# SingleRust/single-algebra

Hardware: AMD Instinct MI355X
Metric: sparse_pca_fit_transform_algorithmic_throughput (higher is better)
Workload: dtype f32

## Files before the change

### single-algebra_amd/csrc/common.h

```cpp
#pragma once
#include <hip/hip_runtime.h>

#include <atomic>
#include <cstdint>
#include <cstdio>
#include <stdexcept>
#include <string>
#include <vector>

#include "../../include/sapca.h"
#include "switches.h"

namespace sapca {

struct Error : std::runtime_error {
  sapca_status code;
  Error(sapca_status c, const std::string& m) : std::runtime_error(m), code(c) {}
};

#define SAPCA_HIP(expr)                                                                        \
  do {                                                                                         \
    hipError_t e_ = (expr);                                                                    \
    if (e_ != hipSuccess)                                                                      \
      throw ::sapca::Error(SAPCA_ERR_HIP, std::string(#expr) + ": " + hipGetErrorString(e_)); \
  } while (0)

#define SAPCA_CHECK(cond, code, msg)                 \
  do {                                               \
    if (!(cond)) throw ::sapca::Error((code), (msg)); \
  } while (0)

inline int64_t round_up(int64_t x, int64_t q) { return (x + q - 1) / q * q; }

struct DevBuf {
  void* p = nullptr;
  size_t cap = 0;
  DevBuf() = default;
  DevBuf(const DevBuf&) = delete;
  DevBuf& operator=(const DevBuf&) = delete;
  ~DevBuf() { release(); }
  void release() {
    if (p) (void)hipFree(p);
    p = nullptr;
    cap = 0;
  }
  void* ensure(size_t bytes) {
    if (bytes > cap) {
      release();
      size_t want = bytes + bytes / 16 + 256;
      hipError_t e = hipMalloc(&p, want);
      if (e != hipSuccess) {
        p = nullptr;
        throw Error(SAPCA_ERR_NOMEM, std::string("hipMalloc(") + std::to_string(want) + "): " + hipGetErrorString(e));
      }
      cap = want;
    }
    return p;
  }
  template <typename U>
  U* as(size_t count) { return static_cast<U*>(ensure(count * sizeof(U))); }
// ... 48 lines not shown
      cap = bytes;
    }
    return p;
  }
};

struct TiledOp {
  bool valid = false;
  int64_t rows = 0, cols = 0, total_entries = 0;
  int ldp = 0;
  int elem = 4;
  int tc = 0, nct = 0;
  int nrb = 0;
  int block_rows = 0;
  int nsplit = 1, tiles_per_split = 0;
  int tile_bytes = 0;
  int64_t max_chunk = 0;
  const int32_t* blk_row0 = nullptr;
  int64_t mid_row0 = -1;
  const uint32_t* row_perm = nullptr;
  const int64_t* chunk_off = nullptr;
  const uint32_t* wave_off = nullptr;
  const uint8_t* steps = nullptr;
  const void* ent = nullptr;
  bool dq = false;
  const uint32_t* dq_info = nullptr;
};
struct TiledBuffers {
  DevBuf blk, steps, wave_off, chunk_off, ent, tmp, misc, perm, lens, dq_info, bounds;
  DevBuf seg;
  DevBuf quad_off;
  DevBuf raw;
  PinnedBuf host;
  hipStream_t aux = nullptr;
  hipEvent_t aux_fork = nullptr, aux_join = nullptr;
  TiledBuffers() = default;
  TiledBuffers(const TiledBuffers&) = delete;
  TiledBuffers& operator=(const TiledBuffers&) = delete;
  ~TiledBuffers() {
    if (aux) { (void)hipStreamSynchronize(aux); (void)hipStreamDestroy(aux); }
    if (aux_fork) (void)hipEventDestroy(aux_fork);
    if (aux_join) (void)hipEventDestroy(aux_join);
  }
};

struct Stream {
  hipStream_t s = nullptr;
  bool owned = false;
};

struct EventTimer {
  bool enabled = false;
  hipStream_t s = nullptr;
  std::vector<std::pair<hipEvent_t, hipEvent_t>> pool;
  size_t used = 0;
  struct Span { size_t i; };
  void begin_collect(hipStream_t st, bool on) {
    enabled = on;
    s = st;
    used = 0;
  }
  int start() {
    if (!enabled) return -1;
    if (used == pool.size()) {
      hipEvent_t a, b;
      SAPCA_HIP(hipEventCreate(&a));
      SAPCA_HIP(hipEventCreate(&b));
      pool.emplace_back(a, b);
    }
    SAPCA_HIP(hipEventRecord(pool[used].first, s));
    return (int)used++;
  }
  void stop(int i) {
    if (i >= 0) SAPCA_HIP(hipEventRecord(pool[i].second, s));
  }
  double ms(int i) {
    if (i < 0) return 0.0;
    float t = 0;
    SAPCA_HIP(hipEventElapsedTime(&t, pool[i].first, pool[i].second));
    return t;
  }
  ~EventTimer() {
    for (auto& p : pool) {
      (void)hipEventDestroy(p.first);
      (void)hipEventDestroy(p.second);
    }
  }
};

}
```

### single-algebra_amd/csrc/dense.hip

```cpp
#include "kernels.h"

#include <algorithm>
#include <cmath>
#include <vector>

namespace sapca {
namespace k {

namespace {

constexpr int WAVE = 64;
typedef double d4 __attribute__((ext_vector_type(4)));

__device__ inline d4 mfma_f64(double a, double b, d4 c) { return __builtin_amdgcn_mfma_f64_16x16x4f64(a, b, c, 0, 0, 0); }

template <typename T, int NT>
__global__ void __launch_bounds__(256)
gram_kernel(const T* __restrict__ P, int64_t rows, int ld, double* __restrict__ slabs, const T* __restrict__ Pb = nullptr) {
  constexpr int NPAIR = NT * (NT + 1) / 2;
  extern __shared__ double lds[];
  const int lane = threadIdx.x & (WAVE - 1);
  const int wave = threadIdx.x / WAVE;
  const int g = lane >> 4, c = lane & 15;
  d4 acc[NPAIR];
// ... 121 lines not shown
    const double2 a = *reinterpret_cast<const double2*>(p);
    const double2 b = *reinterpret_cast<const double2*>(p + 2);
    out[0] = a.x; out[1] = a.y; out[2] = b.x; out[3] = b.y;
  }
  __device__ static inline void store(double* p, const double v[4]) {
    *reinterpret_cast<double2*>(p) = make_double2(v[0], v[1]);
    *reinterpret_cast<double2*>(p + 2) = make_double2(v[2], v[3]);
  }
};

template <typename T, int NT, bool SRC, int W>
__device__ __forceinline__ void gramv_wave(T* P, int64_t rows, int ld, double* __restrict__ slab, double* lds,
                                           const PanelSource<T>& src, const T* __restrict__ wgt, int want_sum, int lane, int wave) {
  constexpr int NPAIR = NT * (NT + 1) / 2;
  constexpr bool SPLIT = NT > 6;
  constexpr int MINE = SPLIT ? (NPAIR - W + 3) / 4 : NPAIR;
  constexpr int NH = NT / 4;
  const int g = lane >> 4, c = lane & 15;
  const bool owner = !SPLIT || W == 0;
  d4 acc[MINE];
#pragma unroll
  for (int p = 0; p < MINE; ++p) acc[p] = d4{0, 0, 0, 0};
  double cs[NT];
#pragma unroll
  for (int t = 0; t < NT; ++t) cs[t] = 0;
  const int64_t stride = SPLIT ? (int64_t)gridDim.x * 4 : (int64_t)gridDim.x * 16;
  int64_t r0 = SPLIT ? (int64_t)blockIdx.x * 4 : ((int64_t)blockIdx.x * 4 + wave) * 4;
  auto mma = [&](const T (&x)[NT], double wr) {
    double v[NT];
#pragma unroll
    for (int t = 0; t < NT; ++t) v[t] = (double)x[t];
    if (want_sum && owner) {
#pragma unroll
      for (int t = 0; t < NT; ++t) cs[t] += wr * v[t];
    }
    int p = 0, mine = 0;
#pragma unroll
    for (int ta = 0; ta < NT; ++ta)
#pragma unroll
      for (int tb = ta; tb < NT; ++tb) {
        if (!SPLIT || p % 4 == W) {
          acc[mine] = mfma_f64(v[ta], v[tb], acc[mine]);
          ++mine;
        }
        ++p;
      }
  };
  if constexpr (SRC) {
    T sv[NT];
    if (src.mu) {
#pragma unroll
      for (int hh = 0; hh < NH; ++hh) Four<T>::load(src.sv + 64 * hh + 4 * c, &sv[4 * hh]);
    }
    for (; r0 < rows; r0 += stride) {
      const int64_t r = r0 + g;
      T x[NT];
#pragma unroll
      for (int t = 0; t < NT; ++t) x[t] = (T)0;
      double wr = 0;
      if (r < rows) {
        const T* p = src.parts + r * ld + 4 * c;
#pragma unroll
        for (int hh = 0; hh < NH; ++hh) Four<T>::load(p + 64 * hh, &x[4 * hh]);
        for (int sp = 1; sp < src.nsplit; ++sp) {
          T y[NT];
#pragma unroll
          for (int hh = 0; hh < NH; ++hh) Four<T>::load(p + sp * src.slab_stride + 64 * hh, &y[4 * hh]);
#pragma unroll
          for (int t = 0; t < NT; ++t) x[t] += y[t];
        }
        if (src.mu) {
          const T m = src.mu[r];
#pragma unroll
          for (int t = 0; t < NT; ++t) x[t] -= m * sv[t];
        }
        if (owner) {
#pragma unroll
          for (int hh = 0; hh < NH; ++hh) Four<T>::store(P + r * ld + 64 * hh + 4 * c, &x[4 * hh]);
        }
        wr = wgt ? (double)wgt[r] : 1.0;
      }
      mma(x, wr);
    }
  } else {
    constexpr int D = NT == 4 ? 4 : 2;
    T buf[D][NT];
    double wb[D];
    auto fetch = [&](int64_t r, T (&out)[NT], double& wr) {
      if (r < rows) {
#pragma unroll
        for (int hh = 0; hh < NH; ++hh) Four<T>::load(P + r * ld + 64 * hh + 4 * c, &out[4 * hh]);
        wr = (want_sum && wgt) ? (double)wgt[r] : 1.0;
      } else {
#pragma unroll
        for (int t = 0; t < NT; ++t) out[t] = (T)0;
        wr = 0;
      }
    };
#pragma unroll
    for (int d = 0; d < D; ++d) fetch(r0 + d * stride + g, buf[d], wb[d]);
    for (; r0 < rows; r0 += D * stride) {
#pragma unroll
      for (int d = 0; d < D; ++d) {
        T x[NT];
#pragma unroll
        for (int t = 0; t < NT; ++t) x[t] = buf[d][t];
        const double wr = wb[d];
        fetch(r0 + (d + D) * stride + g, buf[d], wb[d]);
        mma(x, wr);
      }
    }
  }
  if (want_sum && owner) {
#pragma unroll
    for (int t = 0; t < NT; ++t) {
      cs[t] += __shfl_xor(cs[t], 16);
      cs[t] += __shfl_xor(cs[t], 32);
    }
  }
  if constexpr (SPLIT) {
#pragma unroll
    for (int q = 0; q < MINE; ++q)
#pragma unroll
      for (int reg = 0; reg < 4; ++reg) slab[((W + 4 * q) * 4 + reg) * WAVE + lane] = acc[q][reg];
    if (owner && g == 0) {
#pragma unroll
      for (int t = 0; t < NT; ++t) slab[NPAIR * 256 + 16 * t + c] = want_sum ? cs[t] : 0.0;
    }
  } else {
    double* lsum = lds + NPAIR * 256;
    for (int w = 0; w < 4; ++w) {
      if (wave == w) {
#pragma unroll
        for (int p = 0; p < NPAIR; ++p)
#pragma unroll
          for (int reg = 0; reg < 4; ++reg) {
            double* dst = lds + (p * 4 + reg) * WAVE + lane;
            if (w == 0) *dst = acc[p][reg]; else *dst += acc[p][reg];
          }
        if (g == 0) {
#pragma unroll
          for (int t = 0; t < NT; ++t) {
            double* dst = lsum + 16 * t + c;
            if (w == 0) *dst = cs[t]; else *dst += cs[t];
          }
        }
      }
      __syncthreads();
    }
    for (int i = threadIdx.x; i < NPAIR * 256 + 16 * NT; i += blockDim.x) slab[i] = lds[i];
  }
}

template <typename T, int NT, bool SRC>
__global__ void __launch_bounds__(256)
gramv_kernel(T* P, int64_t rows, int ld, double* __restrict__ slabs, PanelSource<T> src, const T* __restrict__ wgt, int want_sum) {
  constexpr int NPAIR = NT * (NT + 1) / 2;
  extern __shared__ double lds[];
  const int lane = threadIdx.x & (WAVE - 1), wave = threadIdx.x / WAVE;
  double* slab = slabs + (int64_t)blockIdx.x * (NPAIR * 256 + 16 * NT);
  if constexpr (NT > 6) {
    switch (wave) {
      case 0: gramv_wave<T, NT, SRC, 0>(P, rows, ld, slab, lds, src, wgt, want_sum, lane, wave); break;
      case 1: gramv_wave<T, NT, SRC, 1>(P, rows, ld, slab, lds, src, wgt, want_sum, lane, wave); break;
      case 2: gramv_wave<T, NT, SRC, 2>(P, rows, ld, slab, lds, src, wgt, want_sum, lane, wave); break;
      default: gramv_wave<T, NT, SRC, 3>(P, rows, ld, slab, lds, src, wgt, want_sum, lane, wave); break;
    }
  } else {
    gramv_wave<T, NT, SRC, 0>(P, rows, ld, slab, lds, src, wgt, want_sum, lane, wave);
  }
}

template <typename T>
__global__ void materialize_kernel(T* P, int64_t rows, int ld, PanelSource<T> src) {
  const int64_t total = rows * ld;
  int64_t i = (int64_t)blockIdx.x * blockDim.x + threadIdx.x;
  const int64_t stride = (int64_t)gridDim.x * blockDim.x;
  for (; i < total; i += stride) {
    T x = src.parts[i];
    for (int sp = 1; sp < src.nsplit; ++sp) x += src.parts[(int64_t)sp * src.slab_stride + i];
    if (src.mu) x -= src.mu[i / ld] * src.sv[i % ld];
    P[i] = x;
  }
}

template <typename T>
__global__ void rinv_tvec_kernel(const double* __restrict__ Rinv, int l, int ld, const double* __restrict__ wsum, T* __restrict__ vec) {
  const int j = blockIdx.x * blockDim.x + threadIdx.x;
  if (j >= ld) return;
  double s = 0;
  if (j < l)
    for (int i = 0; i <= j; ++i) s += Rinv[(size_t)i * ld + j] * wsum[i];
  vec[j] = (T)s;
}

__global__ void __launch_bounds__(256)
gram_reduce_kernel(const double* __restrict__ slabs, int nslabs, int nt, int ld, double* __restrict__ G, int vtiles = 0,
                   double* __restrict__ wsum = nullptr) {
  __shared__ double part[16][17];
  const int npair = nt * (nt + 1) / 2;
  const int slab_len = npair * 256 + (vtiles ? 16 * nt : 0);
  const int e = threadIdx.x & 15, grp = threadIdx.x >> 4;
  const int i = blockIdx.x * 16 + e;
  double sum = 0;
  if (i < slab_len)
    for (int b = grp; b < nslabs; b += 16) sum += slabs[(int64_t)b * slab_len + i];
  part[grp][e] = sum;
  __syncthreads();
  if (grp != 0 || i >= slab_len) return;
  sum = 0;
#pragma unroll
  for (int g2 = 0; g2 < 16; ++g2) sum += part[g2][e];
  if (i >= npair * 256) {
    const int t = (i - npair * 256) / 16, c = (i - npair * 256) % 16;
    if (wsum) wsum[vcol(t, c)] = sum;
    return;
  }
  int p = i / 256, rem = i % 256, reg = rem / 64, lane = rem % 64;
  int ta = 0;
  while (p >= nt - ta) { p -= nt - ta; ++ta; }
  const int tb = ta + p;
  const int row = vtiles ? vcol(ta, (lane >> 4) + 4 * reg) : 16 * ta + (lane >> 4) + 4 * reg;
  const int col = vtiles ? vcol(tb, lane & 15) : 16 * tb + (lane & 15);
  G[row * ld + col] = sum;
  G[col * ld + row] = sum;
}

__global__ void __launch_bounds__(256)
chol_inv_kernel(const double* __restrict__ G, int l, int ld, double* __restrict__ R, double* __restrict__ Rinv,
                int* __restrict__ info) {
  extern __shared__ double a[];
  const int st = l + 1;
  double* dinv = a + (size_t)l * st;
  __shared__ int bad;
  __shared__ double floor_s;
  const int tid = threadIdx.x;
  const int ti = tid >> 4, tj = tid & 15;
  if (tid == 0) bad = 0;
  for (int i = tid; i < l * l; i += blockDim.x) a[(i / l) * st + (i % l)] = G[(i / l) * ld + (i % l)];
  __syncthreads();
  if (tid == 0) {
    double scale = 0;
    for (int i = 0; i < l; ++i) scale = fmax(scale, fabs(a[i * st + i]));
    floor_s = scale * 1e-13 + 1e-300;
  }
  __syncthreads();
  for (int kk = 0; kk < l; ++kk) {
    if (tid == 0) {
      double v = a[kk * st + kk];
      if (!(v > floor_s)) { v = floor_s; bad += 1; }
      v = sqrt(v);
      a[kk * st + kk] = v;
      dinv[kk] = 1.0 / v;
    }
    __syncthreads();
    const double inv = dinv[kk];
    for (int j = kk + 1 + tid; j < l; j += blockDim.x) a[kk * st + j] *= inv;
    __syncthreads();
    for (int i = kk + 1 + ti; i < l; i += 16) {
// ... 317 lines not shown
  }
  __syncthreads();
  chol_inv_core<false>(B0, B2, dinvs, nb2, floor_s, bad);
#pragma unroll
  for (int u = 0; u < 16; ++u) {
    const int e = t + u * 256, r = e >> 6, c = e & 63;
    const bool in = r < l2 && c < l2 && c >= r;
    R[(size_t)(CHN + r) * LD + CHN + c] = in ? B0[c * CHP + r] : 0.0;
    Rinv[(size_t)(CHN + r) * LD + CHN + c] = in ? B2[c * CHP + r] : 0.0;
  }
  __syncthreads();
  for (int blk = wave; blk < 16; blk += 4) {
    const int I = blk >> 2, J = blk & 3;
    const d4 acc = mm_block(B3 + I * CHB * CHP + J * CHB, CHP, 1, B1 + J * CHB * CHP + J * CHB, CHP, 1, 4 - J, lane);
#pragma unroll
    for (int reg = 0; reg < 4; ++reg) B0[(I * CHB + g4 + 4 * reg) * CHP + J * CHB + i16] = acc[reg];
  }
  __syncthreads();
  for (int blk = wave; blk < 16; blk += 4) {
    const int I = blk >> 2, J = blk & 3;
    const d4 acc = mm_block(B2 + I * CHB * CHP, CHP, 1, B0 + J * CHB, CHP, 1, I + 1, lane);
#pragma unroll
    for (int reg = 0; reg < 4; ++reg) B3[(I * CHB + g4 + 4 * reg) * CHP + J * CHB + i16] = -acc[reg];
  }
  __syncthreads();
#pragma unroll
  for (int u = 0; u < 16; ++u) {
    const int e = t + u * 256, r = e >> 6, c = e & 63;
    Rinv[(size_t)r * LD + CHN + c] = c < l2 ? B3[c * CHP + r] : 0.0;
  }
  if (t == 0 && bad) atomicAdd(info, bad);
}

template <typename T> struct Quad;
template <> struct Quad<float> {
  __device__ static inline void load(const float* p, double out[4]) {
    const float4 v = *reinterpret_cast<const float4*>(p);
    out[0] = v.x; out[1] = v.y; out[2] = v.z; out[3] = v.w;
  }
};
template <> struct Quad<double> {
  __device__ static inline void load(const double* p, double out[4]) {
    const double2 a = *reinterpret_cast<const double2*>(p);
    const double2 b = *reinterpret_cast<const double2*>(p + 2);
    out[0] = a.x; out[1] = a.y; out[2] = b.x; out[3] = b.y;
  }
};

template <typename T, int NTO, int THREADS = 256>
__global__ void __launch_bounds__(THREADS, THREADS == 512 ? 4 : 1)
panel_gemm_kernel(const T* P, int64_t rows, int ld, const double* __restrict__ M, int ldo, T* out, int ldp_stride, int ldm_stride,
                  int ldo_stride, int accumulate, int upper, int ncols_out) {
  extern __shared__ double Ms[];
  for (int i = threadIdx.x; i < ld * ldo; i += blockDim.x) Ms[i] = M[(i / ldo) * ldm_stride + (i % ldo)];
  __syncthreads();
  const int lane = threadIdx.x & (WAVE - 1);
  const int wave = threadIdx.x / WAVE;
  const int i = lane & 15, g = lane >> 4;
  const int nt = ld / 16;
  const int64_t ntiles = (rows + 15) / 16;
  constexpr int WPB = THREADS / WAVE;
  for (int64_t tile = (int64_t)blockIdx.x * WPB + wave; tile < ntiles; tile += (int64_t)gridDim.x * WPB) {
    const int64_t r0 = tile * 16;
    const bool row_ok = r0 + i < rows;
    const T* prow = P + (row_ok ? (r0 + i) : 0) * ldp_stride + 4 * g;
    d4 acc[NTO];
#pragma unroll
    for (int tb = 0; tb < NTO; ++tb) acc[tb] = d4{0, 0, 0, 0};
    for (int j = 0; j < nt; ++j) {
      double a4[4] = {0, 0, 0, 0};
      if (row_ok) Quad<T>::load(prow + 16 * j, a4);
#pragma unroll
      for (int e = 0; e < 4; ++e) {
        const double* brow = Ms + (16 * j + 4 * g + e) * ldo + i;
#pragma unroll
        for (int tb = 0; tb < NTO; ++tb)
          if (!upper || tb + upper - 1 >= j) acc[tb] = mfma_f64(a4[e], brow[16 * tb], acc[tb]);
      }
    }
#pragma unroll
    for (int tb = 0; tb < NTO; ++tb)
#pragma unroll
      for (int reg = 0; reg < 4; ++reg) {
        const int64_t r = r0 + g + 4 * reg;
        if (r < rows && 16 * tb + i < ncols_out) {
          T* o = out + r * ldo_stride + 16 * tb + i;
          *o = accumulate ? (T)((double)*o + acc[tb][reg]) : (T)acc[tb][reg];
        }
      }
  }
}

constexpr int EIG_THREADS = 1024;
constexpr int EIG_MAX_L = 112;
constexpr int EIG_MAX_SWEEPS = 40;

__device__ __forceinline__ int eig_tri(int i, int j, int l) {
  return i * l - (i * (i - 1)) / 2 + (j - i);
}

__global__ void __launch_bounds__(EIG_THREADS)
sym_eig_jacobi_kernel(const double* __restrict__ G, int l, int ld, int k, int ldk, double* __restrict__ M, double* __restrict__ sigma_out,
                      int* __restrict__ status) {
  extern __shared__ double eig_lds[];
  const int L = (l + 1) & ~1;
  const int np = L / 2;
  const int vs = l | 1;
// ... 325 lines not shown

inline int grid_for(int64_t work_items, int block, int cap = 4096) {
  int64_t g = (work_items + block - 1) / block;
  if (g < 1) g = 1;
  if (g > cap) g = cap;
  return (int)g;
}

template <typename T>
static void colsum_f64(const T* P, int64_t rows, int ld, const T* w, double* out, double* partial, hipStream_t s) {
  int by = 256 / ld;
  if (by < 1) by = 1;
  int nblocks = (int)((rows + by * 8 - 1) / (by * 8));
  if (nblocks > 1024) nblocks = 1024;
  if (nblocks < 1) nblocks = 1;
  hipLaunchKernelGGL((colsum_partial_kernel<T>), dim3(nblocks), dim3(ld, by), (size_t)by * ld * sizeof(double), s, P, rows, ld, w, partial);
  hipLaunchKernelGGL((colsum_final_kernel<double>), dim3(ld), dim3(64), 0, s, partial, nblocks, ld, out);
}

template <typename T, int NT>
void launch_gram(const T* P, int64_t rows, int ld, double* slabs, int nblocks, hipStream_t s) {
  constexpr int NPAIR = NT * (NT + 1) / 2;
  if constexpr (NT >= 7) {
    hipLaunchKernelGGL((gram_split_kernel<T, NT>), dim3(nblocks), dim3(256), 0, s, P, rows, ld, slabs, (const T*)nullptr);
    return;
  }
  const size_t lds = (size_t)NPAIR * 256 * sizeof(double);
  static LdsAttrState attr;
  if (lds > 48 * 1024) ensure_dynamic_lds(reinterpret_cast<const void*>(&gram_kernel<T, NT>), lds, attr);
  hipLaunchKernelGGL((gram_kernel<T, NT>), dim3(nblocks), dim3(256), lds, s, P, rows, ld, slabs);
}

template <typename T, int NTO>
void launch_panel_gemm(const T* P, int64_t rows, int ld, const double* M, int ldo, T* out, hipStream_t s, int ldp_stride = 0,
                       int ldm_stride = 0, int ldo_stride = 0, int accumulate = 0, int upper = 0, int ncols_out = 0) {
  if (ncols_out <= 0 || ncols_out > ldo) ncols_out = ldo;
  const size_t lds = (size_t)ld * ldo * sizeof(double);
  static LdsAttrState attr;
  if (lds > 48 * 1024) ensure_dynamic_lds(reinterpret_cast<const void*>(&panel_gemm_kernel<T, NTO>), lds, attr);
  const int64_t ntiles = (rows + 15) / 16;
  if constexpr (NTO >= 7) {
    if (lds > 80 * 1024) {
      static LdsAttrState attr12;
      ensure_dynamic_lds(reinterpret_cast<const void*>(&panel_gemm_kernel<T, NTO, 768>), lds, attr12);
      int blocks = (int)((ntiles + 11) / 12);
      if (blocks > 256) blocks = 256;
      if (blocks < 1) blocks = 1;
      hipLaunchKernelGGL((panel_gemm_kernel<T, NTO, 768>), dim3(blocks), dim3(768), lds, s, P, rows, ld, M, ldo, out, ldp_stride ? ldp_stride : ld,
                         ldm_stride ? ldm_stride : ldo, ldo_stride ? ldo_stride : ldo, accumulate, upper, ncols_out);
      return;
    }
  }
  if constexpr (NTO == 4) {
    if (ntiles >= 4096) {
      static LdsAttrState attr8;
      if (lds > 48 * 1024) ensure_dynamic_lds(reinterpret_cast<const void*>(&panel_gemm_kernel<T, NTO, 512>), lds, attr8);
      int blocks = (int)((ntiles + 7) / 8);
      if (blocks > 1024) blocks = 1024;
      hipLaunchKernelGGL((panel_gemm_kernel<T, NTO, 512>), dim3(blocks), dim3(512), lds, s, P, rows, ld, M, ldo, out, ldp_stride ? ldp_stride : ld,
                         ldm_stride ? ldm_stride : ldo, ldo_stride ? ldo_stride : ldo, accumulate, upper, ncols_out);
      return;
    }
  }
  int blocks = (int)((ntiles + 3) / 4);
  if (blocks > 1024) blocks = 1024;
  if (blocks < 1) blocks = 1;
  hipLaunchKernelGGL((panel_gemm_kernel<T, NTO>), dim3(blocks), dim3(256), lds, s, P, rows, ld, M, ldo, out, ldp_stride ? ldp_stride : ld,
                     ldm_stride ? ldm_stride : ldo, ldo_stride ? ldo_stride : ldo, accumulate, upper, ncols_out);
}

}

__global__ void gram_place_pair_kernel(const double* __restrict__ G2, int bi, int bj, int ld, double* __restrict__ G) {
  const int i = blockIdx.x * blockDim.x + threadIdx.x;
  if (i >= 128 * 128) return;
  const int r = i / 128, c = i % 128;
  const int gr = (r < 64 ? 64 * bi : 64 * bj - 64) + r, gc = (c < 64 ? 64 * bi : 64 * bj - 64) + c;
  G[(int64_t)gr * ld + gc] = G2[i];
}

template <typename T, int NT>
static void launch_gramv(T* P, int64_t rows, int ld, double* slabs, int nblocks, const PanelSource<T>* src, const T* w, bool want_sum,
                         hipStream_t s) {
  constexpr int NPAIR = NT * (NT + 1) / 2;
  const size_t lds = NT > 6 ? 0 : (size_t)(NPAIR * 256 + 16 * NT) * sizeof(double);
  if (src) {
    hipLaunchKernelGGL((gramv_kernel<T, NT, true>), dim3(nblocks), dim3(256), lds, s, P, rows, ld, slabs, *src, w, want_sum ? 1 : 0);
  } else {
    hipLaunchKernelGGL((gramv_kernel<T, NT, false>), dim3(nblocks), dim3(256), lds, s, P, rows, ld, slabs, PanelSource<T>{}, w, want_sum ? 1 : 0);
  }
}

template <typename T>
void materialize(T* P, int64_t rows, int ld, const PanelSource<T>& src, hipStream_t s) {
  if (rows == 0 || (src.parts == P && src.nsplit <= 1 && !src.mu)) return;
  hipLaunchKernelGGL((materialize_kernel<T>), dim3(grid_for(rows * ld, 256)), dim3(256), 0, s, P, rows, ld, src);
  SAPCA_HIP(hipGetLastError());
}

template <typename T>
void gram(T* P, int64_t rows, int ld, double* G, DevBuf& scratch, hipStream_t s, const PanelSource<T>* src, const T* w, double* wsum) {
  SAPCA_CHECK(ld % 16 == 0 && ld >= 16 && (ld <= 128 || (ld % 64 == 0 && ld <= kMaxPanelWidth)), SAPCA_ERR_ARG,
              "gram: panel width must be a multiple of 16 up to 128, or of 64 up to 1024");
  const int nt = ld / 16;
  if (nt == 4 || nt == 8) {
    if (src && nt == 8 && src->parts == P) {
      materialize(P, rows, ld, *src, s);
// ... 323 lines not shown
```

### single-algebra_amd/csrc/engine.cpp

```cpp
#include "engine.h"

#include <algorithm>
#include <chrono>
#include <cmath>
#include <cstring>
#include <exception>
#include <memory>
#include <thread>

#include "lanczos.h"
#include "small_svd.h"
#include "spmm_dq.h"

namespace sapca {

namespace {

template <typename T>
int staged_sweep_ldp(int64_t rows, int64_t cols, double entries, int64_t l, int spmm_variant) {
  if (spmm_variant == 1 || rows <= 0 || cols <= 0 || l < 1 || l > k::kMaxPanelWidth) return 0;
  const int ldp = 64;
  const double row_bytes = (double)ldp * sizeof(T);
  const double tile_bytes = 80.0 * 1024.0, block_rows = row_bytes == 256.0 ? 512.0 : 256.0;
  const double chunks = std::ceil((double)rows / block_rows) * std::ceil((double)cols * row_bytes / tile_bytes);
  double floor_entries = sizeof(T) == 4 ? 1e7 : 5e6;
  if (const char* e = dbg_env("SAPCA_TILED_MIN_ENTRIES")) floor_entries = atof(e);
  const bool dense_enough = entries * (sizeof(T) == 4 ? 64.0 : 96.0) >= chunks * tile_bytes && entries >= floor_entries;
  return (spmm_variant == 2 || dense_enough) ? ldp : 0;
}

enum Cat { C_PREPARE, C_STATS, C_SPMM, C_SPMMT, C_ORTHO, C_SMALL, C_LANCZOS, C_TRANSFORM, C_COMM, C_COUNT };

struct Scope {
  sapca_handle_s& h;
  int ev;
  Scope(sapca_handle_s& h_, int cat) : h(h_), ev(h_.timer.start()) {
    if (ev >= 0) h.spans.emplace_back(cat, ev);
  }
  ~Scope() {
    try { h.timer.stop(ev); } catch (...) {}
  }
};

void collect_timings(sapca_handle_s& h, bool is_fit) {
  if (!h.timer.enabled) return;
  sapca_timings& t = h.timings;
  if (is_fit) {
    const double keep_upload = t.upload_ms;
    const uint64_t keep_steps = t.lanczos_steps;
    std::memset(&t, 0, sizeof(t));
    t.upload_ms = keep_upload;
    t.lanczos_steps = keep_steps;
  } else {
    t.transform_ms = 0;
    for (int ev : h.held_small.in_transform) t.transform_ms -= h.timer.ms(ev);
  }
  double comm_dev_ms = 0;
  for (auto& sp : h.spans) {
    if (is_fit == (sp.first == C_TRANSFORM)) continue;
    const double ms = h.timer.ms(sp.second);
    switch (sp.first) {
      case C_PREPARE: t.prepare_ms += ms; break;
      case C_STATS: t.stats_ms += ms; break;
      case C_SPMM:
        t.spmm_ms += ms;
        if (t.n_spmm < 32) t.spmm_sweep_ms[t.n_spmm] = ms;
        t.n_spmm++;
        break;
      case C_SPMMT:
        t.spmmt_ms += ms;
        if (t.n_spmmt < 32) t.spmmt_sweep_ms[t.n_spmmt] = ms;
        t.n_spmmt++;
        break;
      case C_ORTHO: t.ortho_ms += ms; break;
      case C_SMALL: t.small_svd_ms += ms; break;
      case C_LANCZOS: t.lanczos_ms += ms; break;
      case C_TRANSFORM: t.transform_ms += ms; break;
      case C_COMM: comm_dev_ms += ms; break;
      default: break;
    }
  }
  if (is_fit) t.comm_ms = comm_dev_ms > 0 ? comm_dev_ms : h.comm.host_ms;
}

using H = sapca_handle_s;

void lazy_stream(hipStream_t& st, hipEvent_t& a, hipEvent_t& b) {
  if (st) return;
  SAPCA_HIP(hipStreamCreateWithFlags(&st, hipStreamNonBlocking));
// ... 385 lines not shown
    out.a_aside = true;
  }

  column_statistics(h, A, p, out);
  if (!p.masked) {
    h.a_used = {p.m, p.n, p.nnz, A.ptr, A.idx, A.val};
    h.at_used = {p.n, p.m, p.nnz, out.At.ptr, out.At.idx, out.At.val};
  } else if (lz_scatter) {
    h.at_used = {p.n_used, p.m, out.nnz_used, nullptr, nullptr, nullptr};
  }

  build_formats(h, p, out, aside);
  aside.join();
  if (out.a_aside) SAPCA_HIP(hipStreamWaitEvent(s, h.ev_join, 0));
  if (p.deliver == StatsTo::SideChain) queue_side_statistics(h, p, out, maps);

  h.prep_key = prep_key_of(h, A);
}

template <typename T>
void Engine<T>::finish_statistics(H& h) {
  const int64_t n = h.stats_cols;
  const double* sums = static_cast<const double*>(h.stats_host.p);
  const double mg = (double)h.m_global;
  const bool masked = h.has_mask_maps;
  h.prep_mean.assign((size_t)n, 0.0);
  h.prep_total_var = 0;
  if (h.opt.center) {
    for (int64_t j = 0; j < n; ++j) h.prep_mean[(size_t)j] = (double)(T)(sums[(size_t)j] / mg);
    auto var_of = [&](int64_t j) {
      const double mean = sums[(size_t)j] / mg;
      return (sums[(size_t)n + j] - mean * sums[(size_t)j]) / (mg - 1.0);
    };
    if (masked) for (uint64_t j : h.cols_to_use) h.prep_total_var += var_of((int64_t)j);
    else for (int64_t j = 0; j < n; ++j) h.prep_total_var += var_of(j);
  }
  h.q3_cancels = false;
  if (h.opt.center && masked)
    for (uint64_t j : h.cols_to_use) {
      const double sj = sums[(size_t)j], qj = sums[(size_t)n + j];
      if (qj > 0 && sj * sj > 0.25 * mg * qj) { h.q3_cancels = true; break; }
    }
  h.stats_pending = false;
}

template <typename T>
void Engine<T>::normalize(H& h, T* P, int64_t rows, int l, int ld, int normalizer, bool sharded, const NormalizeExtras<T>& x) {
  hipStream_t s = h.stream;
  if (normalizer == SAPCA_NORM_NONE) {
    if (x.src) k::materialize(P, rows, ld, *x.src, s);
    if (x.vec_out) k::weighted_colsum(P, rows, ld, x.w, x.vec_out, h.scratch2, s);
    return;
  }
  Scope sc(h, C_ORTHO);
  const SmallLayout lay(h.small, ld);
  double *G = lay.gram(), *wsum = x.vec_out ? lay.wsum() : nullptr;
  const int passes = x.passes > 0 ? x.passes : (normalizer == SAPCA_NORM_QR ? 2 : 1);
  for (int pass = 0; pass < passes; ++pass) {
    k::gram(P, rows, ld, G, h.scratch2, s, pass == 0 ? x.src : nullptr, x.w, wsum);
    if (sharded && h.comm.active()) { Scope cs(h, C_COMM); h.comm.allreduce(G, (uint64_t)ld * ld, 1, s); }
    double* Rout = pass == 0 ? x.R1 : x.R2;
    k::chol_inv(G, l, ld, Rout ? Rout : lay.r_scratch(), lay.r_inv(), lay.info(), s, wsum,
                sizeof(T) == 4 ? reinterpret_cast<float*>(x.vec_out) : nullptr, sizeof(T) == 8 ? reinterpret_cast<double*>(x.vec_out) : nullptr);
    T* Q = ld <= 128 ? P : h.panel_wide.as<T>((size_t)std::max<int64_t>(rows, 1) * ld);
    k::panel_gemm(P, rows, ld, lay.r_inv(), ld, Q, s, true);
    if (Q != P) SAPCA_HIP(hipMemcpyAsync(P, Q, (size_t)rows * ld * sizeof(T), hipMemcpyDeviceToDevice, s));
  }
}

template <typename T>
bool Engine<T>::vote_rides(const H& h) {
  return sizeof(T) == 4 && h.comm.active() && h.opt.method == SAPCA_RANDOM && h.opt.spmm_variant != 1 &&
         (size_t)h.comm.nranks + 2 <= H::kStatsTail;
}

template <typename T>
int64_t Engine<T>::piece_vote(H& h, int ld) {
  const char* ov = getenv("SAPCA_AT_OVERLAP");
  const bool enabled = ov != nullptr ? atoi(ov) != 0 : h.comm.mode != Comm::RCCL;
  if (!enabled || !h.comm.has_side_lane() || !k::spmm_tiled_pieces_ok(h.tiled_at, 2, ld)) return 0;
  std::vector<int64_t> b;
  k::spmm_tiled_piece_bounds(h.tiled_at, 2, b, h.stream);
  return b[1];
}

namespace {

enum class AtSweep { OnePiece, TwoPieces };
enum class SmallSvd { GramHost, GramHostHeldBack, GramDevice, QrJacobi };

struct AtPieces {
  AtSweep sweep = AtSweep::OnePiece;
  int64_t cut = 0, r1 = 0;
  int wgs = 240;
};
struct RandomizedPlan {
  int64_t m = 0, n_used = 0;
  int l = 0, ld = 0, k = 0, ldk = 0, q = 0;
  int norm = 0, variant = 0;
  bool center = false, tiled = false;
  bool cov = false;
  bool scale = false;
  SmallSvd small = SmallSvd::GramHost;
  AtPieces at;
};

template <typename T>
// ... 29 lines not shown

template <typename T>
AtPieces agree_on_at_pieces(H& h, const RandomizedPlan& p) {
  AtPieces at;
  h.at_sweep_pieces = 1u;
  if (sizeof(T) != 4 || !h.comm.active() || p.variant == 1) return at;
  hipStream_t s = h.stream;
  const bool mine = h.tiled_at.valid && k::spmm_tiled_pieces_ok(h.tiled_at, 2, p.ld);
  if (h.vote_ready) {
    at.cut = h.vote_cut;
    SAPCA_CHECK(at.cut == 0 || mine, SAPCA_ERR_COMM, "internal: the ranks agreed on a two-piece A^T sweep this rank cannot run");
  } else {
    const uint32_t nr = h.comm.nranks;
    std::vector<double> votes((size_t)nr, 0.0);
    votes[h.comm.rank] = mine ? (double)Engine<T>::piece_vote(h, p.ld) : 0.0;
    double* d_votes = h.votes.as<double>(nr);
    SAPCA_HIP(hipMemcpyAsync(d_votes, votes.data(), nr * sizeof(double), hipMemcpyHostToDevice, s));
    h.comm.allreduce(d_votes, nr, 1, s);
    SAPCA_HIP(hipMemcpyAsync(votes.data(), d_votes, nr * sizeof(double), hipMemcpyDeviceToHost, s));
    SAPCA_HIP(hipStreamSynchronize(s));
    at.cut = (int64_t)*std::min_element(votes.begin(), votes.end());
  }
  if (!mine || at.cut <= 0 || at.cut >= p.n_used) return at;
  std::vector<int64_t> piece_rows;
  k::spmm_tiled_piece_bounds(h.tiled_at, 2, piece_rows, s);
  at.sweep = AtSweep::TwoPieces;
  at.r1 = piece_rows[1];
  h.at_sweep_pieces = 2u;
  hipDeviceProp_t pr;
  if (hipGetDeviceProperties(&pr, h.device) == hipSuccess) at.wgs = std::max(16, pr.multiProcessorCount - 16);
  lazy_stream(h.stream_comm, h.ev_piece, h.ev_comm);
  return at;
}

template <typename T>
void load_omega(H& h, const RandomizedPlan& p, FitPanels<T>& f) {
  hipStream_t s = h.stream;
  if (h.omega.empty()) {
    k::gaussian_panel(f.X, p.n_used, p.l, p.ld, h.opt.random_seed, s);
    return;
  }
  SAPCA_CHECK((int64_t)h.omega_rows == p.n_used && (int64_t)h.omega_cols >= p.l, SAPCA_ERR_ARG,
              "injected Omega must be (features seen by the SVD) x (n_components + n_oversamples)");
  std::vector<T> tmp((size_t)p.n_used * p.l);
  for (int64_t r = 0; r < p.n_used; ++r)
    for (int j = 0; j < p.l; ++j) tmp[(size_t)r * p.l + j] = (T)h.omega[(size_t)r * h.omega_cols + j];
  T* stage = h.scratch2.as<T>(tmp.size());
  SAPCA_HIP(hipMemcpyAsync(stage, tmp.data(), tmp.size() * sizeof(T), hipMemcpyHostToDevice, s));
  k::add_padding(stage, p.n_used, p.l, f.X, p.ld, s);
  SAPCA_HIP(hipStreamSynchronize(s));
}

template <typename T>
void sweep_a(H& h, const RandomizedPlan& p, FitPanels<T>& f) {
  hipStream_t s = h.stream;
  if (p.scale) {
    Scope sc(h, C_ORTHO);
    k::scale_panel_rows(f.X, p.n_used, p.ld, f.d, s);
  }
  if (p.center && !f.cvec_current) k::weighted_colsum(f.X, p.n_used, p.ld, f.mu, f.cvec, h.scratch2, s);
  f.cvec_current = false;
  Scope sc(h, C_SPMM);
  k::spmm(Engine<T>::view(h.a_used), &h.tiled_a, f.X, p.ld, f.Y, p.ld, p.ld, p.center ? f.cvec : nullptr, p.variant, h.split_scratch, s);
}

template <typename T>
double* covar_s(H& h, int ld) { return h.covar_s.as<double>((size_t)k::kCovarCols * (size_t)std::max(ld, 16)); }

template <typename T>
void covar_basis_sweep(H& h, const RandomizedPlan& p, FitPanels<T>& f) {
  hipStream_t s = h.stream;
  constexpr int kq = k::kCovarCols;
  T* Q = h.covar_q.as<T>((size_t)p.m * kq);
  SAPCA_HIP(hipMemcpyAsync(Q, h.covar.q_t.data(), (size_t)p.m * kq * sizeof(T), hipMemcpyHostToDevice, s));
  T* Gp = h.panel_xs.as<T>(((size_t)std::max<int64_t>(p.n_used, 1) + 1) * p.ld);
  T* G = h.covar_g.as<T>((size_t)p.n_used * kq);
  k::add_padding(Q, p.m, kq, f.Y, p.ld, s);
  {
    Scope sc(h, C_SPMMT);
    k::spmm(Engine<T>::view(h.at_used), &h.tiled_at, f.Y, p.ld, Gp, p.ld, p.ld, (const T*)nullptr, p.variant, h.split_scratch, s);
  }
  k::strip_padding(Gp, p.n_used, p.ld, kq, G, s);
  if (p.scale) k::scale_panel_rows(G, p.n_used, kq, f.d, s);
}

template <typename T>
void covar_model_products(H& h, const RandomizedPlan& p) {
  hipStream_t s = h.stream;
  constexpr int kq = k::kCovarCols;
  Scope sc(h, C_ORTHO);
  const int ldc = (int)round_up(p.k, p.k > 128 ? 64 : 16);
  h.covar.ldc = ldc;
  T* W = h.panel_w.as<T>((size_t)std::max<int64_t>(p.n_used, 1) * ldc);
  double* C = h.covar_c.as<double>((size_t)kq * ldc);
  double* GG = covar_s<T>(h, kq);
  const T* G = h.covar_g.ptr<T>();
  k::scaled_transpose(h.components_dev.ptr<T>(), p.n_used, p.k, nullptr, W, ldc, s);
  k::panel_qt_y(W, G, p.n_used, ldc, C, h.scratch2, s);
  k::panel_qt_y(G, G, p.n_used, kq, GG, h.scratch2, s);
  void* host = h.covar_host.ensure((size_t)kq * kq * sizeof(double));
  SAPCA_HIP(hipMemcpyAsync(host, GG, (size_t)kq * kq * sizeof(double), hipMemcpyDeviceToHost, s));
}

template <typename T>
void covar_project(H& h, const RandomizedPlan& p, FitPanels<T>& f, bool behind_at) {
  Scope sc(h, C_ORTHO);
  double* S = covar_s<T>(h, p.ld);
  k::panel_qt_y(f.Y, h.covar_q.ptr<T>(), p.m, p.ld, S, h.scratch2, h.stream);
  if (behind_at) k::panel_sub_qs(f.X, h.covar_g.ptr<T>(), p.n_used, p.ld, p.ld, S, p.ld, h.stream);
  else k::panel_sub_qs(f.Y, h.covar_q.ptr<T>(), p.m, p.ld, p.ld, S, p.ld, h.stream);
}

template <typename T>
void sweep_at_one_piece(H& h, const RandomizedPlan& p, FitPanels<T>& f) {
  hipStream_t s = h.stream;
  f.src = k::PanelSource<T>();
  {
    Scope sc(h, C_SPMMT);
    k::spmm(Engine<T>::view(h.at_used), &h.tiled_at, f.Y, p.ld, f.X, p.ld, p.ld, (const T*)nullptr, p.variant, h.split_scratch, s,
            h.comm.active() || p.cov ? nullptr : &f.src);
  }
  if (!f.src.parts) { f.src.parts = f.X; f.src.nsplit = 1; }
  if (h.comm.active()) {
    Scope cs(h, C_COMM);
    h.comm.allreduce(f.X, (uint64_t)p.n_used * p.ld + (p.center ? (uint64_t)p.ld : 0), Engine<T>::kDtype, s);
  }
  if (p.center) { f.src.mu = f.mu; f.src.sv = f.sv; }
}

template <typename T>
void sweep_at_two_pieces(H& h, const RandomizedPlan& p, FitPanels<T>& f) {
  if constexpr (sizeof(T) == 4) {
    hipStream_t s = h.stream;
    const int64_t cut = p.at.cut, r1 = p.at.r1;
    f.src = k::PanelSource<T>();
    {
      Scope sc(h, C_SPMMT);
      k::spmm_tiled_piece(h.tiled_at, 0, 2, p.at.wgs, 0, r1, f.Y, p.ld, f.X, p.ld, p.ld, h.split_scratch, s);
      SAPCA_HIP(hipEventRecord(h.ev_piece, s));
      k::spmm_tiled_piece(h.tiled_at, 1, 2, p.at.wgs, r1, p.n_used - r1, f.Y, p.ld, f.X, p.ld, p.ld, h.split_scratch2, s);
    }
    Scope cs(h, C_COMM);
    SAPCA_HIP(hipStreamWaitEvent(h.stream_comm, h.ev_piece, 0));
    h.comm.allreduce(f.X, (uint64_t)cut * p.ld, Engine<T>::kDtype, h.stream_comm, 1);
    SAPCA_HIP(hipEventRecord(h.ev_comm, h.stream_comm));
    h.comm.allreduce(f.X + (size_t)cut * p.ld, (uint64_t)(p.n_used - cut) * p.ld + (p.center ? (uint64_t)p.ld : 0), Engine<T>::kDtype, s);
    SAPCA_HIP(hipStreamWaitEvent(s, h.ev_comm, 0));
    f.src.parts = f.X; f.src.nsplit = 1;
    if (p.center) { f.src.mu = f.mu; f.src.sv = f.sv; }
  }
}

template <typename T>
void sweep_at(H& h, const RandomizedPlan& p, FitPanels<T>& f) {
  p.at.sweep == AtSweep::TwoPieces ? sweep_at_two_pieces(h, p, f) : sweep_at_one_piece(h, p, f);
  if (p.scale) {
    Scope sc(h, C_ORTHO);
    k::finish_scaled_panel(f.X, p.n_used, p.ld, f.src, f.d, h.stream);
    f.src = k::PanelSource<T>();
    f.src.parts = f.X; f.src.nsplit = 1;
  }
  if (p.cov) covar_project(h, p, f, true);
}

template <typename T>
void power_iterations(H& h, const RandomizedPlan& p, FitPanels<T>& f) {
  using Extras = NormalizeExtras<T>;
  T* const sv_out = p.center ? f.sv : nullptr;
  for (int it = 0; it < p.q; ++it) {
    sweep_a(h, p, f);
    if (p.cov) covar_project(h, p, f, false);
    Engine<T>::normalize(h, f.Y, p.m, p.l, p.ld, p.norm, true, Extras{.passes = 1, .vec_out = sv_out});
    sweep_at(h, p, f);
    Engine<T>::normalize(h, f.X, p.n_used, p.l, p.ld, p.norm, false,
                         Extras{.passes = 1, .src = &f.src, .w = p.scale ? f.dmu : f.mu, .vec_out = p.center ? f.cvec : nullptr});
    f.cvec_current = p.center;
  }
  sweep_a(h, p, f);
  if (p.cov) covar_project(h, p, f, false);
  Engine<T>::normalize(h, f.Y, p.m, p.l, p.ld, SAPCA_NORM_QR, true, Extras{.vec_out = sv_out});
  sweep_at(h, p, f);
}

template <typename T>
void rotate_into_components(H& h, int ld, const double* Mdev, const double** sign_out = nullptr) {
  const int k = (int)h.opt.n_components, ldk = (int)round_up(k, 16);
  const int64_t n_used = h.a_used.cols;
  T* VtT = h.panel_w.as<T>((size_t)std::max<int64_t>(n_used, 1) * ldk);
  k::panel_gemm(h.panel_x.ptr<T>(), n_used, ld, Mdev, ldk, VtT, h.stream);
  T* comps = h.components_dev.as<T>((size_t)k * std::max<int64_t>(n_used, 1));
  k::flip_transpose(VtT, n_used, ldk, k, comps, h.scratch2, h.stream, sign_out);
}

template <typename T>
void small_svd_gram_device(H& h, const RandomizedPlan& p, FitPanels<T>& f) {
  hipStream_t s = h.stream;
  Scope sc(h, C_SMALL);
  k::gram(f.X, p.n_used, p.ld, f.lay.gram(), h.scratch2, s, &f.src);
  double* d_sigma = f.lay.r_inv();
  int* d_status = reinterpret_cast<int*>(d_sigma + p.ld);
  k::sym_eig_device(f.lay.gram(), p.l, p.ld, p.k, p.ldk, f.lay.m(), d_sigma, d_status, s);
  double* host = static_cast<double*>(h.small_host.ensure(((size_t)p.l + 4) * sizeof(double)));
  int* host_i = reinterpret_cast<int*>(host + p.l);
  SAPCA_HIP(hipMemcpyAsync(host, d_sigma, (size_t)p.l * sizeof(double), hipMemcpyDeviceToHost, s));
  SAPCA_HIP(hipMemcpyAsync(host_i, d_status, 2 * sizeof(int), hipMemcpyDeviceToHost, s));
  SAPCA_HIP(hipMemcpyAsync(host_i + 2, f.lay.info(), sizeof(int), hipMemcpyDeviceToHost, s));
  rotate_into_components<T>(h, p.ld, f.lay.m());
  h.held_tail.sing_l = p.l;
}

template <typename T>
void small_svd_gram_host(H& h, const RandomizedPlan& p, FitPanels<T>& f) {
  hipStream_t s = h.stream;
  Scope sc(h, C_SMALL);
  k::gram(f.X, p.n_used, p.ld, f.lay.gram(), h.scratch2, s, &f.src);
  const size_t g_len = (size_t)p.ld * p.ld, m_len = (size_t)p.ld * p.ldk;
  double* g = static_cast<double*>(h.small_host.ensure((g_len + m_len + 2) * sizeof(double)));
  int* info_pinned = reinterpret_cast<int*>(g + g_len + m_len);
  SAPCA_HIP(hipMemcpyAsync(g, f.lay.gram(), g_len * sizeof(double), hipMemcpyDeviceToHost, s));
  SAPCA_HIP(hipMemcpyAsync(info_pinned, f.lay.info(), sizeof(int), hipMemcpyDeviceToHost, s));
  h.held_small.l = p.l;
  h.held_small.ld = p.ld;
  if (p.small == SmallSvd::GramHostHeldBack) {
    if (!h.held_small.ev) SAPCA_HIP(hipEventCreateWithFlags(&h.held_small.ev, hipEventDisableTiming));
    SAPCA_HIP(hipEventRecord(h.held_small.ev, s));
    h.held_small.pending = true;
    return;
  }
  Engine<T>::finish_small_svd(h, nullptr);
}

template <typename T>
void small_svd_qr_jacobi(H& h, const RandomizedPlan& p, FitPanels<T>& f) {
  hipStream_t s = h.stream;
// ... 521 lines not shown
```

### single-algebra_amd/csrc/engine.h

```cpp
#pragma once
#include <algorithm>
#include <string>
#include <vector>

#include "comm.h"
#include "common.h"
#include "kernels.h"

struct sapca_handle_s {
  sapca_options opt{};
  std::string err;
  int device = 0;
  hipStream_t stream = nullptr;
  bool own_stream = false;
  hipStream_t stream2 = nullptr;
  hipEvent_t ev_fork = nullptr, ev_join = nullptr, ev_drop = nullptr;
  hipStream_t stream3 = nullptr;
  hipStream_t stream_comm = nullptr;
  hipEvent_t ev_piece = nullptr, ev_comm = nullptr;
  hipEvent_t ev_kept = nullptr, ev_stats = nullptr;
  bool stats_on_side = false;

  std::vector<uint8_t> mask;
  uint64_t mask_version = 0;
// ... 138 lines not shown
  sapca::Comm comm;
};

namespace sapca {

struct SmallLayout {
  size_t ld, W;
  double* base;
  SmallLayout(DevBuf& buf, int ld_, size_t behind = 0)
      : ld((size_t)ld_), W((size_t)std::max(ld_, 128)), base(buf.as<double>(6 * W * W + 64 + 4 * W + behind)) {}
  double* slot(size_t i) const { return base + i * ld * ld; }
  double* gram() const { return slot(0); }
  double* r_inv() const { return slot(1); }
  double* r_scratch() const { return slot(2); }
  double* r1() const { return slot(3); }
  double* r2() const { return slot(4); }
  double* m() const { return slot(5); }
  int* info() const { return reinterpret_cast<int*>(base + 6 * W * W); }
  template <typename T> T* c() const { return reinterpret_cast<T*>(base + 6 * W * W + 64); }
  template <typename T> T* s() const { return c<T>() + W; }
  double* wsum() const { return base + 6 * W * W + 64 + 2 * W; }
  double* behind() const { return base + 6 * W * W + 64 + 4 * W; }
};

template <typename T>
struct CsrBuf {
  int64_t* ptr; int32_t* idx; T* val;
  sapca_handle_s::RawCsr raw(int64_t rows, int64_t cols, int64_t nnz) const { return {rows, cols, nnz, ptr, idx, val}; }
};
template <typename T>
CsrBuf<T> csr_buffers(DevBuf& ptr, DevBuf& idx, DevBuf& val, int64_t rows, int64_t cap) {
  const size_t entries = (size_t)std::max<int64_t>(cap, 1);
  return {ptr.as<int64_t>((size_t)rows + 1), idx.as<int32_t>(entries), val.as<T>(entries)};
}

template <typename T>
CsrView<T> transpose_into_at(sapca_handle_s& h, const CsrView<T>& A) {
  h.prep_key.valid = false;
  const CsrBuf<T> at = csr_buffers<T>(h.at_ptr, h.at_idx, h.at_val, A.cols, A.nnz);
  k::transpose_csr(A, at.ptr, at.idx, at.val, h.scratch, h.stream);
  return CsrView<T>{A.cols, A.rows, A.nnz, at.ptr, at.idx, at.val};
}

void covar_check(sapca_handle_s& h, uint64_t m, bool fit, bool then_transform);
void scale_check(sapca_handle_s& h, uint64_t m, uint64_t n, bool fit, bool then_transform);

template <typename T>
struct NormalizeExtras {
  double *R1 = nullptr, *R2 = nullptr;
  int passes = 0;
  const k::PanelSource<T>* src = nullptr;
  const T* w = nullptr;
  T* vec_out = nullptr;
};

template <typename T>
struct Engine {
  using H = sapca_handle_s;
  static constexpr int kDtype = sizeof(T) == 8 ? 1 : 0;
  static void prepare(H& h, const CsrView<T>& A);
  static void finish_statistics(H& h);
  static void fit(H& h, const CsrView<T>& A, bool defer_finish = false);
  static void finish_small_svd(H& h, const double** sign_out);
  static void finish_fit(H& h);
  static void transform(H& h, const CsrView<T>& A, T* d_out);
  static void fit_randomized(H& h);
  static void fit_lanczos(H& h, bool centred);
  static bool vote_rides(const H& h);
  static int64_t piece_vote(H& h, int ld);
  static void normalize(H& h, T* P, int64_t rows, int l, int ld, int normalizer, bool sharded, const NormalizeExtras<T>& x);
  static CsrView<T> view(const H::RawCsr& r) {
    CsrView<T> v;
    v.rows = r.rows; v.cols = r.cols; v.nnz = r.nnz;
    v.ptr = static_cast<const int64_t*>(r.ptr);
    v.idx = static_cast<const int32_t*>(r.idx);
    v.val = static_cast<const T*>(r.val);
    return v;
  }
};

}
```

Baseline: 1343.

## Prefetch next-row slabs in gram kernel, unroll reductions, share timer events

The panel-source gram kernel now software-pipelines its work: it loads the next row's split slabs, mean and weight ahead of time and accumulates the slabs U at a time. The slab reduction and the panel_gemm LDS fill are unrolled by 8 so more loads are in flight. gramv_kernel gets a launch-bounds occupancy hint of 2 blocks, and the 8-tile panel_gemm path now applies from a lower tile count. Separately, the event timer reuses the previous span's stop event as the next span's start, which cuts hipEventRecord calls between back-to-back stages. The trade-off is higher register pressure from the prefetch buffers, which the launch-bounds hint may turn into spills.

```diff
diff --git a/single-algebra_amd/csrc/common.h b/single-algebra_amd/csrc/common.h
--- a/single-algebra_amd/csrc/common.h
+++ b/single-algebra_amd/csrc/common.h
@@ -6,6 +6,7 @@
 #include <cstdio>
 #include <stdexcept>
 #include <string>
+#include <utility>
 #include <vector>
 
 #include "../../include/sapca.h"
@@ -160,39 +161,50 @@
 struct EventTimer {
   bool enabled = false;
   hipStream_t s = nullptr;
-  std::vector<std::pair<hipEvent_t, hipEvent_t>> pool;
+  std::vector<hipEvent_t> pool;
   size_t used = 0;
-  struct Span { size_t i; };
+  std::vector<std::pair<int, int>> spans;
+  int last_closed = -1;
   void begin_collect(hipStream_t st, bool on) {
     enabled = on;
     s = st;
     used = 0;
+    spans.clear();
+    last_closed = -1;
+  }
+  int record() {
+    if (used == pool.size()) {
+      hipEvent_t e;
+      SAPCA_HIP(hipEventCreate(&e));
+      pool.push_back(e);
+    }
+    SAPCA_HIP(hipEventRecord(pool[used], s));
+    return (int)used++;
   }
   int start() {
     if (!enabled) return -1;
-    if (used == pool.size()) {
-      hipEvent_t a, b;
-      SAPCA_HIP(hipEventCreate(&a));
-      SAPCA_HIP(hipEventCreate(&b));
-      pool.emplace_back(a, b);
-    }
-    SAPCA_HIP(hipEventRecord(pool[used].first, s));
-    return (int)used++;
+    spans.emplace_back(record(), -1);
+    return (int)spans.size() - 1;
+  }
+  int start_behind_last() {
+    if (!enabled) return -1;
+    if (last_closed < 0) return start();
+    spans.emplace_back(spans[(size_t)last_closed].second, -1);
+    return (int)spans.size() - 1;
   }
   void stop(int i) {
-    if (i >= 0) SAPCA_HIP(hipEventRecord(pool[i].second, s));
+    if (i < 0) return;
+    spans[(size_t)i].second = record();
+    last_closed = i;
   }
   double ms(int i) {
-    if (i < 0) return 0.0;
+    if (i < 0 || spans[(size_t)i].second < 0) return 0.0;
     float t = 0;
-    SAPCA_HIP(hipEventElapsedTime(&t, pool[i].first, pool[i].second));
+    SAPCA_HIP(hipEventElapsedTime(&t, pool[(size_t)spans[(size_t)i].first], pool[(size_t)spans[(size_t)i].second]));
     return t;
   }
   ~EventTimer() {
-    for (auto& p : pool) {
-      (void)hipEventDestroy(p.first);
-      (void)hipEventDestroy(p.second);
-    }
+    for (hipEvent_t e : pool) (void)hipEventDestroy(e);
   }
 };
 
diff --git a/single-algebra_amd/csrc/dense.hip b/single-algebra_amd/csrc/dense.hip
--- a/single-algebra_amd/csrc/dense.hip
+++ b/single-algebra_amd/csrc/dense.hip
@@ -197,25 +197,73 @@
 #pragma unroll
       for (int hh = 0; hh < NH; ++hh) Four<T>::load(src.sv + 64 * hh + 4 * c, &sv[4 * hh]);
     }
+    constexpr int U = NT * sizeof(T) <= 16 ? 4 : NT * sizeof(T) <= 32 ? 2 : 1;
+    const int nsplit = src.nsplit;
+    const int64_t ss = src.slab_stride;
+    auto load_slab = [&](const T* p, int sp, T (&y)[NT]) {
+#pragma unroll
+      for (int hh = 0; hh < NH; ++hh) Four<T>::load(p + sp * ss + 64 * hh, &y[4 * hh]);
+    };
+    T hx[NT], hy[U][NT], hm = (T)0;
+    double hw = 0;
+    auto head = [&](int64_t r) {
+      if (r < rows) {
+        const T* p = src.parts + r * ld + 4 * c;
+        load_slab(p, 0, hx);
+#pragma unroll
+        for (int u = 0; u < U; ++u)
+          if (1 + u < nsplit) load_slab(p, 1 + u, hy[u]);
+        if (src.mu) hm = src.mu[r];
+        hw = wgt ? (double)wgt[r] : 1.0;
+      }
+    };
+    head(r0 + g);
     for (; r0 < rows; r0 += stride) {
       const int64_t r = r0 + g;
+      const bool live = r < rows;
       T x[NT];
 #pragma unroll
       for (int t = 0; t < NT; ++t) x[t] = (T)0;
       double wr = 0;
-      if (r < rows) {
+      T m = (T)0;
+      if (live) {
         const T* p = src.parts + r * ld + 4 * c;
 #pragma unroll
-        for (int hh = 0; hh < NH; ++hh) Four<T>::load(p + 64 * hh, &x[4 * hh]);
-        for (int sp = 1; sp < src.nsplit; ++sp) {
-          T y[NT];
-#pragma unroll
-          for (int hh = 0; hh < NH; ++hh) Four<T>::load(p + sp * src.slab_stride + 64 * hh, &y[4 * hh]);
-#pragma unroll
-          for (int t = 0; t < NT; ++t) x[t] += y[t];
+        for (int t = 0; t < NT; ++t) x[t] = hx[t];
+#pragma unroll
+        for (int u = 0; u < U; ++u)
+          if (1 + u < nsplit) {
+#pragma unroll
+            for (int t = 0; t < NT; ++t) x[t] += hy[u][t];
+          }
+        m = hm;
+        wr = hw;
+        int sp = 1 + U;
+        for (; sp + U <= nsplit; sp += U) {
+          T y[U][NT];
+#pragma unroll
+          for (int u = 0; u < U; ++u) load_slab(p, sp + u, y[u]);
+#pragma unroll
+          for (int u = 0; u < U; ++u)
+#pragma unroll
+            for (int t = 0; t < NT; ++t) x[t] += y[u][t];
         }
+        if constexpr (U > 1) if (sp < nsplit) {
+          T y[U > 1 ? U - 1 : 1][NT];
+#pragma unroll
+          for (int u = 0; u < U - 1; ++u)
+            if (sp + u < nsplit) load_slab(p, sp + u, y[u]);
+#pragma unroll
+          for (int u = 0; u < U - 1; ++u)
+            if (sp + u < nsplit) {
+#pragma unroll
+              for (int t = 0; t < NT; ++t) x[t] += y[u][t];
+            }
+        }
+      }
+      head(r0 + stride + g);
+      if (live) {
         if (src.mu) {
-          const T m = src.mu[r];
 #pragma unroll
           for (int t = 0; t < NT; ++t) x[t] -= m * sv[t];
         }
@@ -223,7 +271,6 @@
 #pragma unroll
           for (int hh = 0; hh < NH; ++hh) Four<T>::store(P + r * ld + 64 * hh + 4 * c, &x[4 * hh]);
         }
-        wr = wgt ? (double)wgt[r] : 1.0;
       }
       mma(x, wr);
     }
@@ -298,7 +345,7 @@
 }
 
 template <typename T, int NT, bool SRC>
-__global__ void __launch_bounds__(256)
+__global__ void __launch_bounds__(256, 2)
 gramv_kernel(T* P, int64_t rows, int ld, double* __restrict__ slabs, PanelSource<T> src, const T* __restrict__ wgt, int want_sum) {
   constexpr int NPAIR = NT * (NT + 1) / 2;
   extern __shared__ double lds[];
@@ -348,8 +395,17 @@
   const int e = threadIdx.x & 15, grp = threadIdx.x >> 4;
   const int i = blockIdx.x * 16 + e;
   double sum = 0;
-  if (i < slab_len)
-    for (int b = grp; b < nslabs; b += 16) sum += slabs[(int64_t)b * slab_len + i];
+  if (i < slab_len) {
+    int b = grp;
+    for (; b + 16 * 7 < nslabs; b += 16 * 8) {
+      double v[8];
+#pragma unroll
+      for (int u = 0; u < 8; ++u) v[u] = slabs[(int64_t)(b + 16 * u) * slab_len + i];
+#pragma unroll
+      for (int u = 0; u < 8; ++u) sum += v[u];
+    }
+    for (; b < nslabs; b += 16) sum += slabs[(int64_t)b * slab_len + i];
+  }
   part[grp][e] = sum;
   __syncthreads();
   if (grp != 0 || i >= slab_len) return;
@@ -773,7 +829,20 @@
 panel_gemm_kernel(const T* P, int64_t rows, int ld, const double* __restrict__ M, int ldo, T* out, int ldp_stride, int ldm_stride,
                   int ldo_stride, int accumulate, int upper, int ncols_out) {
   extern __shared__ double Ms[];
-  for (int i = threadIdx.x; i < ld * ldo; i += blockDim.x) Ms[i] = M[(i / ldo) * ldm_stride + (i % ldo)];
+  {
+    const int nel = ld * ldo, step = blockDim.x;
+    const bool dense = ldm_stride == ldo;
+    auto at = [&](int i) { return dense ? i : (i / ldo) * ldm_stride + (i % ldo); };
+    int i = threadIdx.x;
+    for (; i + 7 * step < nel; i += 8 * step) {
+      double v[8];
+#pragma unroll
+      for (int u = 0; u < 8; ++u) v[u] = M[at(i + u * step)];
+#pragma unroll
+      for (int u = 0; u < 8; ++u) Ms[i + u * step] = v[u];
+    }
+    for (; i < nel; i += step) Ms[i] = M[at(i)];
+  }
   __syncthreads();
   const int lane = threadIdx.x & (WAVE - 1);
   const int wave = threadIdx.x / WAVE;
@@ -1205,7 +1274,7 @@
     }
   }
   if constexpr (NTO == 4) {
-    if (ntiles >= 4096) {
+    if (ntiles >= 1024) {
       static LdsAttrState attr8;
       if (lds > 48 * 1024) ensure_dynamic_lds(reinterpret_cast<const void*>(&panel_gemm_kernel<T, NTO, 512>), lds, attr8);
       int blocks = (int)((ntiles + 7) / 8);
diff --git a/single-algebra_amd/csrc/engine.cpp b/single-algebra_amd/csrc/engine.cpp
--- a/single-algebra_amd/csrc/engine.cpp
+++ b/single-algebra_amd/csrc/engine.cpp
@@ -34,7 +34,7 @@
 struct Scope {
   sapca_handle_s& h;
   int ev;
-  Scope(sapca_handle_s& h_, int cat) : h(h_), ev(h_.timer.start()) {
+  Scope(sapca_handle_s& h_, int cat, bool behind_last = false) : h(h_), ev(behind_last ? h_.timer.start_behind_last() : h_.timer.start()) {
     if (ev >= 0) h.spans.emplace_back(cat, ev);
   }
   ~Scope() {
@@ -526,7 +526,7 @@
     if (x.vec_out) k::weighted_colsum(P, rows, ld, x.w, x.vec_out, h.scratch2, s);
     return;
   }
-  Scope sc(h, C_ORTHO);
+  Scope sc(h, C_ORTHO, x.behind_sweep);
   const SmallLayout lay(h.small, ld);
   double *G = lay.gram(), *wsum = x.vec_out ? lay.wsum() : nullptr;
   const int passes = x.passes > 0 ? x.passes : (normalizer == SAPCA_NORM_QR ? 2 : 1);
@@ -662,15 +662,18 @@
 }
 
 template <typename T>
-void sweep_a(H& h, const RandomizedPlan& p, FitPanels<T>& f) {
+void sweep_a(H& h, const RandomizedPlan& p, FitPanels<T>& f, bool behind_normalize) {
   hipStream_t s = h.stream;
   if (p.scale) {
-    Scope sc(h, C_ORTHO);
+    Scope sc(h, C_ORTHO, behind_normalize);
     k::scale_panel_rows(f.X, p.n_used, p.ld, f.d, s);
   }
-  if (p.center && !f.cvec_current) k::weighted_colsum(f.X, p.n_used, p.ld, f.mu, f.cvec, h.scratch2, s);
+  if (p.center && !f.cvec_current) {
+    k::weighted_colsum(f.X, p.n_used, p.ld, f.mu, f.cvec, h.scratch2, s);
+    behind_normalize = false;
+  }
   f.cvec_current = false;
-  Scope sc(h, C_SPMM);
+  Scope sc(h, C_SPMM, behind_normalize);
   k::spmm(Engine<T>::view(h.a_used), &h.tiled_a, f.X, p.ld, f.Y, p.ld, p.ld, p.center ? f.cvec : nullptr, p.variant, h.split_scratch, s);
 }
 
@@ -722,11 +725,11 @@
 }
 
 template <typename T>
-void sweep_at_one_piece(H& h, const RandomizedPlan& p, FitPanels<T>& f) {
+void sweep_at_one_piece(H& h, const RandomizedPlan& p, FitPanels<T>& f, bool behind_normalize) {
   hipStream_t s = h.stream;
   f.src = k::PanelSource<T>();
   {
-    Scope sc(h, C_SPMMT);
+    Scope sc(h, C_SPMMT, behind_normalize);
     k::spmm(Engine<T>::view(h.at_used), &h.tiled_at, f.Y, p.ld, f.X, p.ld, p.ld, (const T*)nullptr, p.variant, h.split_scratch, s,
             h.comm.active() || p.cov ? nullptr : &f.src);
   }
@@ -762,8 +765,8 @@
 }
 
 template <typename T>
-void sweep_at(H& h, const RandomizedPlan& p, FitPanels<T>& f) {
-  p.at.sweep == AtSweep::TwoPieces ? sweep_at_two_pieces(h, p, f) : sweep_at_one_piece(h, p, f);
+void sweep_at(H& h, const RandomizedPlan& p, FitPanels<T>& f, bool behind_normalize) {
+  p.at.sweep == AtSweep::TwoPieces ? sweep_at_two_pieces(h, p, f) : sweep_at_one_piece(h, p, f, behind_normalize);
   if (p.scale) {
     Scope sc(h, C_ORTHO);
     k::finish_scaled_panel(f.X, p.n_used, p.ld, f.src, f.d, h.stream);
@@ -777,19 +780,22 @@
 void power_iterations(H& h, const RandomizedPlan& p, FitPanels<T>& f) {
   using Extras = NormalizeExtras<T>;
   T* const sv_out = p.center ? f.sv : nullptr;
+  const bool y_behind = !p.cov, x_behind = !p.cov && !p.scale && !h.comm.active() && p.at.sweep != AtSweep::TwoPieces;
+  const bool normalises = p.norm != SAPCA_NORM_NONE;
   for (int it = 0; it < p.q; ++it) {
-    sweep_a(h, p, f);
+    sweep_a(h, p, f, it > 0 && normalises);
     if (p.cov) covar_project(h, p, f, false);
-    Engine<T>::normalize(h, f.Y, p.m, p.l, p.ld, p.norm, true, Extras{.passes = 1, .vec_out = sv_out});
-    sweep_at(h, p, f);
+    Engine<T>::normalize(h, f.Y, p.m, p.l, p.ld, p.norm, true, Extras{.passes = 1, .vec_out = sv_out, .behind_sweep = y_behind});
+    sweep_at(h, p, f, normalises);
     Engine<T>::normalize(h, f.X, p.n_used, p.l, p.ld, p.norm, false,
-                         Extras{.passes = 1, .src = &f.src, .w = p.scale ? f.dmu : f.mu, .vec_out = p.center ? f.cvec : nullptr});
+                         Extras{.passes = 1, .src = &f.src, .w = p.scale ? f.dmu : f.mu, .vec_out = p.center ? f.cvec : nullptr,
+                                .behind_sweep = x_behind});
     f.cvec_current = p.center;
   }
-  sweep_a(h, p, f);
+  sweep_a(h, p, f, p.q > 0 && normalises);
   if (p.cov) covar_project(h, p, f, false);
-  Engine<T>::normalize(h, f.Y, p.m, p.l, p.ld, SAPCA_NORM_QR, true, Extras{.vec_out = sv_out});
-  sweep_at(h, p, f);
+  Engine<T>::normalize(h, f.Y, p.m, p.l, p.ld, SAPCA_NORM_QR, true, Extras{.vec_out = sv_out, .behind_sweep = y_behind});
+  sweep_at(h, p, f, true);
 }
 
 template <typename T>
diff --git a/single-algebra_amd/csrc/engine.h b/single-algebra_amd/csrc/engine.h
--- a/single-algebra_amd/csrc/engine.h
+++ b/single-algebra_amd/csrc/engine.h
@@ -214,6 +214,7 @@
   const k::PanelSource<T>* src = nullptr;
   const T* w = nullptr;
   T* vec_out = nullptr;
+  bool behind_sweep = false;
 };
 
 template <typename T>
```

Result: faster. 1359, median of 6 (+1.2%).
